# OpenVectorAI/CoFHE

Measured on AMD Instinct MI355X. Metric: ciphertext-ops/sec + HBM GB/s (% roofline), 128x128 matadd, higher is better.
Workload: dtype u32; 1 GPU; ciphertext_matadd 128x128 per GPU (C2), security 128, k 128, |Delta| = 2088 bits, valid ciphertexts of random plaintexts; elements_per_gpu=16384, parallelism=row-shard x1, collective=none

## Files before the change

### __graft_entry__.py

```python
import json
import os
import subprocess
import sys

ROOT = os.path.dirname(os.path.abspath(__file__))
CSRC = os.path.join(ROOT, "cofhe_amd", "csrc")
LIB = os.path.join(ROOT, "cofhe_amd", "libcofhe_hip.so")
HIP_SOURCES = ["cofhe_hip.hip", "abi.hip", "kernels.hpp", "wire.hip", "shard.hip", "wide.hip", "ctx.hpp", "lane.hpp", "mp.hpp", "qf.hpp",
               "form_io.hpp", "layout.hpp", "wide.hpp", "qfw.hpp", "comb.hip", "comb.hpp"]
HIP_OBJECTS = [("part0", "cofhe_hip.hip", ["-DCOFHE_PART=0"]), ("part1", "cofhe_hip.hip", ["-DCOFHE_PART=1"]),
               ("part2", "cofhe_hip.hip", ["-DCOFHE_PART=2"]), ("abi", "abi.hip", []), ("wire", "wire.hip", []), ("shard", "shard.hip", []),
               ("wide", "wide.hip", []), ("comb", "comb.hip", [])]


def _stale(target, deps):
    if not os.path.exists(target):
        return True
    t = os.path.getmtime(target)
    return any(os.path.getmtime(d) > t for d in deps)


def build_library(src_dir, obj_dir, lib, extra_flags=()) -> None:
    hipcc = os.environ.get("HIPCC", "/opt/rocm/bin/hipcc")
    flags = ["--offload-arch=gfx950", "-O2", "-std=c++17", "-fPIC", "-Wno-unused-value"] + list(extra_flags)
    os.makedirs(obj_dir, exist_ok=True)
    jobs = []
    for name, src, extra in HIP_OBJECTS:
        obj = os.path.join(obj_dir, name + ".o")
        jobs.append((obj, subprocess.Popen([hipcc] + flags + extra + ["-c", os.path.join(src_dir, src), "-o", obj], cwd=ROOT)))
    for obj, pr in jobs:
        if pr.wait() != 0:
            raise subprocess.CalledProcessError(pr.returncode, "hipcc -c -> " + obj)
    subprocess.check_call([hipcc, "--offload-arch=gfx950", "-shared", "-fPIC", "-o", lib] + [o for o, _ in jobs] + ["-ldl"], cwd=ROOT)


def build() -> None:
    deps = [os.path.join(CSRC, f) for f in HIP_SOURCES] + [os.path.join(ROOT, "include", "cofhe_hip.h")]
    if _stale(LIB, deps):
        build_library(CSRC, os.path.join(CSRC, "obj"), LIB)
    odir = os.path.join(ROOT, "oracle")
    if _stale(os.path.join(odir, "libcofhe_oracle.so"),
              [os.path.join(odir, "cofhe_oracle.hpp"), os.path.join(odir, "cofhe_oracle_c.cpp")]):
        subprocess.check_call(["make", "-C", odir])
    hdir = os.path.join(ROOT, "cofhe_amd", "host")
    exe = os.path.join(hdir, "local_bench")
    if _stale(exe, [os.path.join(hdir, f) for f in ("local_bench.cpp", "hip_cryptosystem.hpp", "smpc_local.hpp", "tensor.hpp")] + [LIB]):
        subprocess.check_call(["g++", "-std=c++17", "-O2", "-I/opt/conda/include", "-o", exe,
                               os.path.join(hdir, "local_bench.cpp"), "-L" + os.path.join(ROOT, "cofhe_amd"),
                               "-lcofhe_hip", "-l:libgmp.so.10", "-Wl,-rpath,$ORIGIN/.."], cwd=hdir)
    gdir = os.path.join(ROOT, "tests", "gpu_kernels")
    gso = os.path.join(gdir, "liblehmer_gpu.so")
    if _stale(gso, [os.path.join(gdir, "lehmer_gpu.hip"), os.path.join(CSRC, "mp.hpp"), os.path.join(CSRC, "lane.hpp")]):
        subprocess.check_call([os.environ.get("HIPCC", "/opt/rocm/bin/hipcc"), "--offload-arch=gfx950", "-O2", "-std=c++17", "-fPIC", "-shared",
                               "-Wno-unused-value", "-o", gso, os.path.join(gdir, "lehmer_gpu.hip")], cwd=ROOT)
    sys.path.insert(0, ROOT)
    import cofhe_amd
    cofhe_amd.load_library()


def smoke() -> None:
    sys.path.insert(0, ROOT)
    sys.path.insert(0, os.path.join(ROOT, "tests"))
    from cofhe_amd import Engine
    import oracle_lib as O

    def hx(s):
        return -int(s[1:], 16) if s.startswith("-") else int(s, 16)

    g = os.path.join(ROOT, "tests", "golden")
    prm = json.load(open(os.path.join(g, "params_s128_k128.json")))
    vec = json.load(open(os.path.join(g, "vectors_s128_k128.json")))
    d = hx(prm["delta"])
    eng = Engine(d, device=0)
    v = vec["add_valid"]
    t1, t2 = bytes.fromhex(v["ct1"]), bytes.fromhex(v["ct2"])
    out = eng.add_ciphertext_tensors(t1, t2)
    assert out == bytes.fromhex(v["out"]), "HIP add != golden"
    assert out == O.add(d, t1, t2), "HIP add != oracle"
    v = vec["scal_2d"]
    out = eng.scal_ciphertext_tensors(bytes.fromhex(v["s"]), bytes.fromhex(v["cts"]), bytes.fromhex(v["zero"]))
    assert out == bytes.fromhex(v["out"]), "HIP scal matmul != golden"
    print("smoke ok: add_ciphertext_tensors and scal_ciphertext_tensors match golden vectors and oracle")


if __name__ == "__main__":
    build()
    if len(sys.argv) > 1 and sys.argv[1] == "smoke":
        smoke()
```

### cofhe_amd/csrc/mp.hpp

```cpp
#pragma once
#include "lane.hpp"

namespace cofhe {

#if defined(COFHE_HOSTSIM)
struct SimStats { long batches, batch_steps, divsteps, muls, divrems, resolves, bits_gained; };
inline SimStats g_stats;
#define CF_STAT(x) do { if (c.gl == 0) { x; } } while (0)
#else
#define CF_STAT(x) do { } while (0)
#endif

CF_DEV uint32_t opaque(uint32_t v) {
#if defined(COFHE_HOSTSIM)
    asm volatile("" : "+r"(v));
#else
    asm volatile("" : "+v"(v));
#endif
    return v;
}

template <int P>
struct Mp {
    uint32_t v[P][CH];
};

template <int P>
struct SMp {
    Mp<P> m;
    int neg;
};

template <int P>
CF_DEV void mp_zero(Mp<P> &x) {
    CF_UNROLL for (int p = 0; p < P; p++) CF_UNROLL for (int j = 0; j < CH; j++) x.v[p][j] = 0;
}

template <int P>
CF_DEV void mp_set_word(Ctx &c, Mp<P> &x, uint32_t w) {
    mp_zero(x);
    x.v[0][0] = (c.gl == 0) ? w : 0u;
}

template <int Q, int P>
CF_DEV Mp<Q> mp_resize(const Mp<P> &x) {
    Mp<Q> r;
    CF_UNROLL for (int p = 0; p < Q; p++)
        CF_UNROLL for (int j = 0; j < CH; j++) r.v[p][j] = (p < P) ? x.v[p < P ? p : 0][j] : 0u;
    return r;
}

template <int P>
CF_DEV void mp_select(Mp<P> &r, bool take_y, const Mp<P> &x, const Mp<P> &y) {
    CF_UNROLL for (int p = 0; p < P; p++)
        CF_UNROLL for (int j = 0; j < CH; j++) r.v[p][j] = take_y ? y.v[p][j] : x.v[p][j];
}

template <int P>
CF_DEV void mp_swap(Mp<P> &x, Mp<P> &y) {
    CF_UNROLL for (int p = 0; p < P; p++)
        CF_UNROLL for (int j = 0; j < CH; j++) {
            uint32_t t = x.v[p][j];
            x.v[p][j] = y.v[p][j];
            y.v[p][j] = t;
        }
}

template <int P>
CF_DEV bool mp_is_zero(Ctx &c, const Mp<P> &x) {
    uint32_t o = 0;
    CF_UNROLL for (int p = 0; p < P; p++) CF_UNROLL for (int j = 0; j < CH; j++) o |= x.v[p][j];
    return ballot8(c, o != 0) == 0;
}

template <int P>
CF_DEV bool mp_high_planes_zero(Ctx &c, const Mp<P> &x, int from) {
    uint32_t o = 0;
    CF_UNROLL for (int p = 0; p < P; p++)
        CF_UNROLL for (int j = 0; j < CH; j++) o |= (p >= from) ? x.v[p][j] : 0u;
    return ballot8(c, o != 0) == 0;
}

template <int P>
CF_DEV bool mp_is_word(Ctx &c, const Mp<P> &x, uint32_t w) {
    uint32_t o = 0;
    CF_UNROLL for (int p = 0; p < P; p++)
        CF_UNROLL for (int j = 0; j < CH; j++) {
            uint32_t want = (p == 0 && j == 0 && c.gl == 0) ? w : 0u;
            o |= x.v[p][j] ^ want;
        }
    return ballot8(c, o != 0) == 0;
}

template <int P>
CF_DEV int mp_bitlen(Ctx &c, const Mp<P> &x) {
    uint32_t top = x.v[0][0], idx = 0;
    CF_UNROLL for (int p = 0; p < P; p++)
        CF_UNROLL for (int j = 0; j < CH; j++) {
            if (p == 0 && j == 0) continue;
            const uint32_t w = x.v[p][j];
            top = w ? w : top;
            idx = w ? (uint32_t)(p * PLIMBS + j) : idx;
        }
    const uint32_t best = top ? (idx + (uint32_t)c.gl * CH) * 32u + 32u - (uint32_t)clz32(top) : 0u;
    return (int)group_max(c, best);
}

template <int P>
CF_DEV int mp_cmp(Ctx &c, const Mp<P> &x, const Mp<P> &y) {
    uint32_t key = 0;
    CF_UNROLL for (int p = 0; p < P; p++)
        CF_UNROLL for (int j = 0; j < CH; j++) {
            uint32_t a = x.v[p][j], b = y.v[p][j];
            uint32_t k = ((uint32_t)(p * PLIMBS + c.gl * CH + j + 1) << 1) | (a > b ? 1u : 0u);
            key = (a != b) ? k : key;
        }
    uint32_t m = group_max(c, key);
    return m == 0 ? 0 : ((m & 1) ? 1 : -1);
}

template <int P>
CF_DEV uint32_t mp_get_limb(Ctx &c, const Mp<P> &x, int idx) {
    if (idx < 0 || idx >= P * PLIMBS) return 0;
    int p = idx / PLIMBS, w = idx % PLIMBS;
    int lane = w / CH, j = w % CH;
    uint32_t cand = 0;
    CF_UNROLL for (int pp = 0; pp < P; pp++)
        CF_UNROLL for (int jj = 0; jj < CH; jj++) cand = (pp == p && jj == j) ? x.v[pp][jj] : cand;
    return bcast(c, cand, lane);
}

template <int P>
CF_DEV uint64_t mp_bits64(Ctx &c, const Mp<P> &x, int pos) {
    int i0 = pos >> 5, o = pos & 31;
    uint32_t l0 = mp_get_limb(c, x, i0), l1 = mp_get_limb(c, x, i0 + 1), l2 = mp_get_limb(c, x, i0 + 2);
    uint64_t lo = ((uint64_t)l1 << 32) | l0;
    return o ? ((lo >> o) | ((uint64_t)l2 << (64 - o))) : lo;
}
template <int P>
CF_DEV uint32_t mp_bits32(Ctx &c, const Mp<P> &x, int pos) {
    int i0 = pos >> 5, o = pos & 31;
    uint32_t l0 = mp_get_limb(c, x, i0), l1 = mp_get_limb(c, x, i0 + 1);
    return o ? ((l0 >> o) | (l1 << (32 - o))) : l0;
}

template <int P>
CF_DEV uint32_t mp_resolve(Ctx &c, Mp<P> &r, const uint32_t (&hi)[P]) {
    uint32_t plane_word = 0, plane_bit = 0;
    CF_STAT(g_stats.resolves += P);
    CF_UNROLL for (int p = 0; p < P; p++) {
        uint32_t inc = shfl_up1(c, hi[p], plane_word);
        uint64_t t = (uint64_t)r.v[p][0] + inc + ((c.gl == 0) ? plane_bit : 0u);
        r.v[p][0] = (uint32_t)t;
        uint32_t cy = (uint32_t)(t >> 32);
        uint32_t all = r.v[p][0];
        CF_UNROLL for (int j = 1; j < CH; j++) {
            t = (uint64_t)r.v[p][j] + cy;
            r.v[p][j] = (uint32_t)t;
            cy = (uint32_t)(t >> 32);
// ... 60 lines not shown
    uint64_t t[CH];
    CF_UNROLL for (int j = 0; j < CH; j++)
        t[j] = (uint64_t)A * x[j] + (uint64_t)B * (NOTY ? (uint32_t)~y[j] : y[j]);
    uint32_t prev = cin;
#if defined(COFHE_HOSTSIM)
    uint32_t carry = 0;
    CF_UNROLL for (int j = 0; j < CH; j++) {
        const uint64_t s = (uint64_t)(uint32_t)t[j] + prev + carry;
        r[j] = (uint32_t)s;
        carry = (uint32_t)(s >> 32);
        prev = (uint32_t)(t[j] >> 32);
    }
    return prev + carry;
#else
    static_assert(CH == 5, "carry chain written for 5 limbs per lane");
    uint32_t l0 = (uint32_t)t[0], l1 = (uint32_t)t[1], l2 = (uint32_t)t[2], l3 = (uint32_t)t[3], l4 = (uint32_t)t[4];
    const uint32_t h0 = (uint32_t)(t[0] >> 32), h1 = (uint32_t)(t[1] >> 32), h2 = (uint32_t)(t[2] >> 32),
                   h3 = (uint32_t)(t[3] >> 32);
    uint32_t h4 = (uint32_t)(t[4] >> 32);
    asm("v_add_co_u32 %0, vcc, %0, %6\n\t"
        "s_nop 1\n\t"
        "v_addc_co_u32 %1, vcc, %1, %7, vcc\n\t"
        "s_nop 1\n\t"
        "v_addc_co_u32 %2, vcc, %2, %8, vcc\n\t"
        "s_nop 1\n\t"
        "v_addc_co_u32 %3, vcc, %3, %9, vcc\n\t"
        "s_nop 1\n\t"
        "v_addc_co_u32 %4, vcc, %4, %10, vcc\n\t"
        "s_nop 1\n\t"
        "v_addc_co_u32 %5, vcc, 0, %5, vcc"
        : "+v"(l0), "+v"(l1), "+v"(l2), "+v"(l3), "+v"(l4), "+v"(h4)
        : "v"(prev), "v"(h0), "v"(h1), "v"(h2), "v"(h3)
        : "vcc");
    r[0] = l0; r[1] = l1; r[2] = l2; r[3] = l3; r[4] = l4;
    return h4;
#endif
}


template <int P>
CF_DEV uint32_t mp_lincomb_add(Ctx &c, Mp<P> &r, uint32_t A, const Mp<P> &x, uint32_t B, const Mp<P> &y) {
    uint32_t hi[P];
    CF_UNROLL for (int p = 0; p < P; p++) hi[p] = lincomb_plane<false>(r.v[p], A, x.v[p], B, y.v[p], 0u);
    return mp_resolve_sparse(c, r, hi);
}

template <int P>
CF_DEV void mp_lincomb_sub(Ctx &c, Mp<P> &r, uint32_t A, const Mp<P> &x, uint32_t B, const Mp<P> &y) {
    uint32_t hi[P];
    CF_UNROLL for (int p = 0; p < P; p++)
        hi[p] = lincomb_plane<true>(r.v[p], A, x.v[p], B, y.v[p], (p == 0 && c.gl == 0) ? B : 0u);
    (void)mp_resolve(c, r, hi);
}

template <int P>
CF_DEV uint32_t mp_lincomb_sub_carry(Ctx &c, Mp<P> &r, uint32_t A, const Mp<P> &x, uint32_t B, const Mp<P> &y) {
    uint32_t hi[P];
    CF_UNROLL for (int p = 0; p < P; p++)
        hi[p] = lincomb_plane<true>(r.v[p], A, x.v[p], B, y.v[p], (p == 0 && c.gl == 0) ? B : 0u);
    return mp_resolve(c, r, hi);
}

template <int P>
CF_DEV void mp_sub(Ctx &c, Mp<P> &r, const Mp<P> &x, const Mp<P> &y) {
    mp_lincomb_sub(c, r, 1u, x, 1u, y);
}

template <int P>
CF_DEV Mp<P> mp_shl(Ctx &c, const Mp<P> &x, int n) {
    uint32_t *s = c.scratch();
    CF_UNROLL for (int p = 0; p < P; p++)
        CF_UNROLL for (int j = 0; j < CH; j++) s[p * PLIMBS + c.gl * CH + j] = x.v[p][j];
    group_sync(c);
    int w = n >> 5, o = n & 31;
    Mp<P> y;
    CF_UNROLL for (int p = 0; p < P; p++)
        CF_UNROLL for (int j = 0; j < CH; j++) {
            int i = p * PLIMBS + c.gl * CH + j - w;
            uint32_t a = (i >= 0 && i < P * PLIMBS) ? s[i >= 0 && i < P * PLIMBS ? i : 0] : 0u;
            uint32_t b = (i - 1 >= 0 && i - 1 < P * PLIMBS) ? s[i - 1 >= 0 && i - 1 < P * PLIMBS ? i - 1 : 0] : 0u;
            y.v[p][j] = o ? ((a << o) | (b >> (32 - o))) : a;
        }
    group_sync(c);
    return y;
}

template <int P>
CF_DEV Mp<P> mp_shr(Ctx &c, const Mp<P> &x, int n) {
    uint32_t *s = c.scratch();
    CF_UNROLL for (int p = 0; p < P; p++)
        CF_UNROLL for (int j = 0; j < CH; j++) s[p * PLIMBS + c.gl * CH + j] = x.v[p][j];
    group_sync(c);
    int w = n >> 5, o = n & 31;
    Mp<P> y;
    CF_UNROLL for (int p = 0; p < P; p++)
        CF_UNROLL for (int j = 0; j < CH; j++) {
            int i = p * PLIMBS + c.gl * CH + j + w;
            uint32_t a = (i < P * PLIMBS) ? s[i < P * PLIMBS ? i : 0] : 0u;
            uint32_t b = (i + 1 < P * PLIMBS) ? s[i + 1 < P * PLIMBS ? i + 1 : 0] : 0u;
            y.v[p][j] = o ? ((a >> o) | (b << (32 - o))) : a;
        }
    group_sync(c);
    return y;
}

template <int P>
CF_DEV Mp<P> mp_shr_small(Ctx &c, const Mp<P> &x, int n) {
    Mp<P> y;
    uint32_t above = 0;
    const uint32_t ls = (uint32_t)(32 - n) & 31u;
    const uint32_t keep = n ? 0xFFFFFFFFu : 0u;
    CF_UNROLL for (int p = P - 1; p >= 0; p--) {
        uint32_t nxt = shfl_down1(c, x.v[p][0], above);
        CF_UNROLL for (int j = 0; j < CH; j++) {
            uint32_t up = (j + 1 < CH) ? x.v[p][j + 1 < CH ? j + 1 : 0] : nxt;
            y.v[p][j] = (x.v[p][j] >> n) | ((up << ls) & keep);
        }
        above = bcast_first(c, x.v[p][0]);
    }
    return y;
}
template <int P>
CF_DEV Mp<P> mp_shr1(Ctx &c, const Mp<P> &x) { return mp_shr_small(c, x, 1); }

CF_DEV void chunk_mac(uint32_t (&w)[2 * CH + 1], const uint32_t (&x)[CH], const uint32_t (&y)[CH]) {
    CF_UNROLL for (int i = 0; i < CH; i++) {
        uint32_t cy = 0;
        CF_UNROLL for (int j = 0; j < CH; j++) {
            uint64_t m = (uint64_t)x[i] * y[j] + w[i + j] + cy;
            w[i + j] = (uint32_t)m;
            cy = (uint32_t)(m >> 32);
        }
        CF_UNROLL for (int k = i + CH; k < 2 * CH + 1; k++) {
            uint64_t m = (uint64_t)w[k] + cy;
            w[k] = (uint32_t)m;
            cy = (uint32_t)(m >> 32);
        }
    }
}
template <int P, int Q>
CF_DEV Mp<P + Q> mp_mul(Ctx &c, const Mp<P> &x, const Mp<Q> &y) {
    constexpr int R = P + Q;
    CF_STAT(g_stats.muls += P * Q);
    static_assert(R * PLIMBS <= SCRATCH_WORDS && R * G * (CH + 1) <= SCRATCH_WORDS, "scratch too small");
    uint32_t *s = c.scratch();
    CF_UNROLL for (int p = 0; p < P; p++)
        CF_UNROLL for (int j = 0; j < CH; j++) s[p * PLIMBS + c.gl * CH + j] = x.v[p][j];
    CF_UNROLL for (int p = 0; p < Q; p++)
        CF_UNROLL for (int j = 0; j < CH; j++) s[(P + p) * PLIMBS + c.gl * CH + j] = y.v[p][j];
    group_sync(c);
    uint32_t w[R][2 * CH + 1];
    CF_UNROLL for (int p = 0; p < R; p++) CF_UNROLL for (int i = 0; i < 2 * CH + 1; i++) w[p][i] = 0;
    const int ybits = mp_bitlen(c, y);
    CF_UNROLL for (int px = 0; px < P; px++) {
        CF_UNROLL for (int py = 0; py < Q; py++) {
            int ky = (ybits - py * PLIMBS * 32 + CH * 32 - 1) / (CH * 32);
            ky = ky < 0 ? 0 : (ky > G ? G : ky);
            uint32_t cur[2 * CH + 1];
            CF_UNROLL for (int i = 0; i < 2 * CH + 1; i++) cur[i] = w[px + py][i];
            for (int k = 0; k < ky; k++) {
                const bool sw = (k == c.gl + 1);
                CF_UNROLL for (int i = 0; i < 2 * CH + 1; i++) {
                    w[px + py][i] = sw ? cur[i] : w[px + py][i];
                    cur[i] = sw ? w[px + py + 1][i] : cur[i];
                }
                const int lx = (c.gl - k) & (G - 1);
                uint32_t xc[CH], yc[CH];
                CF_UNROLL for (int j = 0; j < CH; j++) {
                    xc[j] = s[(px * G + lx) * CH + j];
                    yc[j] = s[P * PLIMBS + (py * G + k) * CH + j];
                }
                chunk_mac(cur, xc, yc);
            }
            const bool never = (c.gl + 1 >= ky);
            CF_UNROLL for (int i = 0; i < 2 * CH + 1; i++) {
                w[px + py][i] = never ? cur[i] : w[px + py][i];
                w[px + py + 1][i] = never ? w[px + py + 1][i] : cur[i];
            }
        }
    }
    group_sync(c);
    CF_UNROLL for (int p = 0; p < R; p++)
        CF_UNROLL for (int i = 0; i < CH + 1; i++) s[(p * G + c.gl) * (CH + 1) + i] = w[p][CH + i];
    group_sync(c);
    Mp<R> r;
    uint32_t hi[R];
    CF_UNROLL for (int p = 0; p < R; p++) {
        int cc = p * G + c.gl;
        uint32_t cy = 0;
        CF_UNROLL for (int j = 0; j < CH; j++) {
            uint32_t up = (cc >= 1) ? s[(cc >= 1 ? cc - 1 : 0) * (CH + 1) + j] : 0u;
            uint32_t ov = (j == 0 && cc >= 2) ? s[(cc >= 2 ? cc - 2 : 0) * (CH + 1) + CH] : 0u;
            uint64_t t = (uint64_t)w[p][j] + up + ov + cy;
            r.v[p][j] = (uint32_t)t;
            cy = (uint32_t)(t >> 32);
        }
        hi[p] = cy;
    }
    group_sync(c);
    (void)mp_resolve_sparse(c, r, hi);
    return r;
}

CF_DEV uint64_t div64_lower(uint64_t n, uint64_t d) {
    double q = (double)(n & ~0x7FFull) / (double)d;
    uint64_t t = (uint64_t)q;
    return t > 0 ? t - 1 : 0;
}

template <int PN, int PD>
CF_DEV uint32_t mp_quot_digit(Ctx &c, const Mp<PN> &num, int nb, const Mp<PD> &den, int db, int &sh) {
    int npos = nb > 64 ? nb - 64 : 0;
    int dpos = db > 32 ? db - 32 : 0;
    uint64_t nt = mp_bits64(c, num, npos);
    uint64_t dt = (uint64_t)mp_bits32(c, den, dpos) + (dpos > 0 ? 1u : 0u);
    int e = npos - dpos;
    uint64_t t;
    if (CF_UNLIKELY(dt == 0)) {
        CF_STATUS(c, CF_ST_DIV_CAP);
        sh = 0;
        return 1;
    }
    if (dpos == 0 && npos == 0) {
        t = nt / dt;
    } else {
        t = div64_lower(nt, dt);
    }
    if (e < 0) {
        t = (-e >= 64) ? 0 : (t >> (-e));
        e = 0;
    }
    int extra = 33 - __builtin_clzll(t | 1);
    if (extra > 0) {
        t >>= extra;
        e += extra;
    }
    sh = e;
    if (t == 0) {
        sh = 0;
        return 1;
    }
    return (uint32_t)t;
}

template <int PN, int PD>
CF_DEV void mp_divrem_cons(Ctx &c, Mp<PN> &num, const Mp<PD> &den, Mp<PN> &quot) {
    static_assert(PN >= PD, "numerator must be at least as wide as the divisor");
    mp_zero(quot);
    const Mp<PN> dw = mp_resize<PN>(den);
    const int db = mp_bitlen(c, den);
    if (db == 0) {
        CF_STATUS(c, CF_ST_DIV_CAP);
        return;
    }
    for (int guard = 0;; guard++) {
        if (guard > PN * PLIMBS * 32 / 28 + 2) {
            CF_STATUS(c, CF_ST_DIV_CAP);
            break;
        }
        int nb = mp_bitlen(c, num);
        if (nb < db) break;
        if (nb == db && mp_cmp(c, num, dw) < 0) break;
        int sh;
        CF_STAT(g_stats.divsteps++);
        uint32_t qd = mp_quot_digit(c, num, nb, den, db, sh);
        Mp<PN> ds = sh ? mp_shl(c, dw, sh) : dw;
        mp_lincomb_sub(c, num, 1u, num, qd, ds);
        Mp<PN> qa;
        int i0 = sh >> 5, o = sh & 31;
        uint32_t lo = qd << o, hiw = o ? (qd >> (32 - o)) : 0u;
        CF_UNROLL for (int p = 0; p < PN; p++)
            CF_UNROLL for (int j = 0; j < CH; j++) {
                int i = p * PLIMBS + c.gl * CH + j;
                qa.v[p][j] = (i == i0) ? lo : ((i == i0 + 1) ? hiw : 0u);
            }
        (void)mp_add(c, quot, quot, qa);
    }
}

struct WordDiv {
    uint32_t w;
    uint64_t m;
};
CF_DEV uint64_t umulhi64(uint64_t a, uint64_t b) {
#if defined(COFHE_HOSTSIM)
    return (uint64_t)(((unsigned __int128)a * b) >> 64);
#else
    return __umul64hi(a, b);
#endif
}
CF_DEV WordDiv worddiv_make(uint32_t w) {
    WordDiv d;
    d.w = w;
    d.m = ~0ull / w;
    return d;
}
CF_DEV uint64_t worddiv_divmod(const WordDiv &d, uint64_t t, uint32_t &rem) {
    uint64_t q = umulhi64(t, d.m);
    uint64_t r = t - q * d.w;
    while (r >= d.w) {
        r -= d.w;
        q++;
    }
    rem = (uint32_t)r;
    return q;
}
CF_DEV uint32_t worddiv_mulmod(const WordDiv &d, uint32_t a, uint32_t b) {
    uint32_t r;
    (void)worddiv_divmod(d, (uint64_t)a * b, r);
    return r;
}
CF_DEV uint32_t worddiv_addmod(const WordDiv &d, uint32_t a, uint32_t b) {
    uint64_t t = (uint64_t)a + b;
    return (uint32_t)(t >= d.w ? t - d.w : t);
}

template <int P>
CF_DEV uint32_t mp_mod_word(Ctx &c, const Mp<P> &x, const WordDiv &d) {
    uint32_t rem;
    uint32_t two32 = (uint32_t)(0x100000000ull % d.w);
    uint32_t beta = 1;
    CF_UNROLL for (int j = 0; j < CH; j++) beta = worddiv_mulmod(d, beta, two32);
    uint32_t total = 0;
    CF_UNROLL for (int p = P - 1; p >= 0; p--) {
        uint32_t r = 0;
        CF_UNROLL for (int j = CH - 1; j >= 0; j--) {
            (void)worddiv_divmod(d, ((uint64_t)r << 32) | x.v[p][j], rem);
            r = rem;
        }
        uint32_t val = r, wgt = beta;
        CF_UNROLL for (int st = 1; st < G; st <<= 1) {
            uint32_t ov = shfl(c, val, c.gl + st), ow = shfl(c, wgt, c.gl + st);
            bool has = (c.gl + st) < G;
            uint32_t nv = worddiv_addmod(d, worddiv_mulmod(d, ov, wgt), val);
            uint32_t nw = worddiv_mulmod(d, wgt, ow);
            val = has ? nv : val;
            wgt = has ? nw : wgt;
        }
        uint32_t plane_val = bcast_first(c, val), plane_w = bcast_first(c, wgt);
        total = worddiv_addmod(d, worddiv_mulmod(d, total, plane_w), plane_val);
    }
    return total;
}

constexpr uint32_t PRIMORIAL23 = 223092870u;
struct PrimorialWeights { uint32_t w[PLIMBS]; };
constexpr PrimorialWeights primorial_weights() {
    PrimorialWeights t{};
    uint64_t v = 1;
    for (int i = 0; i < PLIMBS; i++) {
        t.w[i] = (uint32_t)v;
        v = (v << 32) % PRIMORIAL23;
    }
    return t;
}
#if defined(COFHE_HOSTSIM)
static constexpr PrimorialWeights PRIMORIAL_W = primorial_weights();
#else
__device__ static constexpr PrimorialWeights PRIMORIAL_W = primorial_weights();
#endif
CF_DEV uint32_t mp_mod_primorial(Ctx &c, const Mp<1> &x) {
    uint64_t acc = 0;
    CF_UNROLL for (int j = 0; j < CH; j++) acc += (uint64_t)x.v[0][j] * PRIMORIAL_W.w[c.gl * CH + j];
    uint32_t v = (uint32_t)(acc % PRIMORIAL23);
    v += shfl_xor1(c, v);
    v += shfl_xor2(c, v);
    v += shfl_mirror(c, v);
    return v % PRIMORIAL23;
}

struct ModW {
    WordDiv dv;
    uint32_t w16[2 * CH];
    uint32_t lanew;
    uint32_t planew;
};
CF_DEV ModW modw_make(Ctx &c, uint32_t W) {
    ModW mw;
    mw.dv = worddiv_make(W);
    uint32_t rem;
    mw.w16[0] = 1u % W;
    CF_UNROLL for (int i = 1; i < 2 * CH; i++) {
        (void)worddiv_divmod(mw.dv, (uint64_t)mw.w16[i - 1] << 16, rem);
        mw.w16[i] = rem;
    }
    (void)worddiv_divmod(mw.dv, (uint64_t)mw.w16[2 * CH - 1] << 16, rem);
    const uint32_t p1 = rem;
    const uint32_t p2 = worddiv_mulmod(mw.dv, p1, p1), p4 = worddiv_mulmod(mw.dv, p2, p2);
    static_assert(G == 8, "lane weights written for 8 lanes per group");
    uint32_t lw = (c.gl & 1) ? p1 : mw.w16[0];
    lw = (c.gl & 2) ? worddiv_mulmod(mw.dv, lw, p2) : lw;
    lw = (c.gl & 4) ? worddiv_mulmod(mw.dv, lw, p4) : lw;
    mw.lanew = lw;
    mw.planew = worddiv_mulmod(mw.dv, p4, p4);
    return mw;
}
template <int P>
CF_DEV uint32_t mp_mod_word_fast(Ctx &c, const Mp<P> &x, const ModW &mw) {
    uint32_t total = 0, rem;
    CF_UNROLL for (int p = P - 1; p >= 0; p--) {
        uint64_t acc = 0;
        CF_UNROLL for (int j = 0; j < CH; j++)
            acc += (uint64_t)(x.v[p][j] & 0xFFFFu) * mw.w16[2 * j] + (uint64_t)(x.v[p][j] >> 16) * mw.w16[2 * j + 1];
        (void)worddiv_divmod(mw.dv, acc, rem);
        uint32_t v = worddiv_mulmod(mw.dv, rem, mw.lanew);
        v = worddiv_addmod(mw.dv, v, shfl_xor1(c, v));
        v = worddiv_addmod(mw.dv, v, shfl_xor2(c, v));
        v = worddiv_addmod(mw.dv, v, shfl_mirror(c, v));
        total = worddiv_addmod(mw.dv, worddiv_mulmod(mw.dv, total, mw.planew), v);
    }
    return total;
}
template <int P>
CF_DEV uint32_t mp_divrem_word(Ctx &c, Mp<P> &num, const WordDiv &d) {
    uint32_t rem;
    uint32_t two32 = (uint32_t)(0x100000000ull % d.w);
    uint32_t beta = 1;
    CF_UNROLL for (int j = 0; j < CH; j++) beta = worddiv_mulmod(d, beta, two32);
    uint32_t above = 0;
    CF_UNROLL for (int p = P - 1; p >= 0; p--) {
        uint32_t r = 0;
        CF_UNROLL for (int j = CH - 1; j >= 0; j--) {
            (void)worddiv_divmod(d, ((uint64_t)r << 32) | num.v[p][j], rem);
            r = rem;
        }
        uint32_t val = r, wgt = beta;
        CF_UNROLL for (int st = 1; st < G; st <<= 1) {
            uint32_t ov = shfl(c, val, c.gl + st), ow = shfl(c, wgt, c.gl + st);
            bool has = (c.gl + st) < G;
            uint32_t nv = worddiv_addmod(d, worddiv_mulmod(d, ov, wgt), val);
            uint32_t nw = worddiv_mulmod(d, wgt, ow);
            val = has ? nv : val;
            wgt = has ? nw : wgt;
        }
        uint32_t hv = shfl_down1(c, val, 0u), hw = shfl_down1(c, wgt, 1u);
        uint32_t h = worddiv_addmod(d, worddiv_mulmod(d, above, hw), hv);
        uint32_t rr = h;
        CF_UNROLL for (int j = CH - 1; j >= 0; j--) {
            uint64_t q = worddiv_divmod(d, ((uint64_t)rr << 32) | num.v[p][j], rem);
            num.v[p][j] = (uint32_t)q;
            rr = rem;
        }
        uint32_t pv = bcast_first(c, val), pw = bcast_first(c, wgt);
        above = worddiv_addmod(d, worddiv_mulmod(d, above, pw), pv);
    }
    return above;
}

template <int PN>
CF_DEV void mp_divrem_norm(Ctx &c, Mp<PN> &num, const Mp<1> &den, int db, Mp<PN> &quot) {
    static_assert(2 * PN * PLIMBS <= SCRATCH_WORDS, "scratch too small");
    mp_zero(quot);
    const int nb = mp_bitlen(c, num);
    if (nb < db) return;
    const int s = PLIMBS * 32 - db;
    const Mp<1> D = s ? mp_shl(c, den, s) : den;
    const uint32_t d39 = bcast_last(c, D.v[0][CH - 1]), d38 = bcast_last(c, D.v[0][CH - 2]);
    const double rd = 1.0 / ((double)d39 * 4294967296.0 + (double)d38);
    uint32_t *sn = c.scratch(), *sq = sn + PN * PLIMBS;
    CF_UNROLL for (int p = 0; p < PN; p++)
        CF_UNROLL for (int j = 0; j < CH; j++) {
            sn[p * PLIMBS + c.gl * CH + j] = num.v[p][j];
            sq[p * PLIMBS + c.gl * CH + j] = 0u;
        }
    group_sync(c);
    const int sw = s >> 5, sb = s & 31;
    auto limb = [&](int k) -> uint32_t {
        const int i = k - sw;
        const uint32_t a = (i >= 0 && i < PN * PLIMBS) ? sn[(i >= 0 && i < PN * PLIMBS) ? i : 0] : 0u;
        const uint32_t b = (i >= 1 && i <= PN * PLIMBS) ? sn[(i >= 1 && i <= PN * PLIMBS) ? i - 1 : 0] : 0u;
        return sb ? ((a << sb) | (b >> (32 - sb))) : a;
    };
    const int K = (nb + s - 1) >> 5;
    Mp<1> S;
    CF_UNROLL for (int j = 0; j < CH; j++) S.v[0][j] = limb(K - (PLIMBS - 1) + c.gl * CH + j);
    uint32_t top = 0;
    for (int k = K - (PLIMBS - 1);; k--) {
        CF_STAT(g_stats.divsteps++);
        const uint32_t l39 = bcast_last(c, S.v[0][CH - 1]), l38 = bcast_last(c, S.v[0][CH - 2]);
        double x = (((double)top * 4294967296.0 + (double)l39) * 4294967296.0 + (double)l38) * rd;
        x += x * 1.7763568394002505e-15;
        uint64_t qd = (uint64_t)x;
        if (qd > 0xFFFFFFFFull) qd = 0xFFFFFFFFull;
        if (CF_LIKELY(qd != 0)) {
            Mp<1> T;
            const uint32_t cw = mp_lincomb_sub_carry(c, T, 1u, S, (uint32_t)qd, D);
            int64_t nt = (int64_t)top + (int64_t)cw - (int64_t)qd;
            S = T;
            for (int fix = 0; CF_UNLIKELY(nt < 0) && fix < 4; fix++) {
                CF_FLAG(8u);
                nt += (int64_t)mp_add(c, S, S, D);
                qd--;
            }
        }
        if (c.gl == 0) sq[k] = (uint32_t)qd;
        if (k == 0) break;
        top = bcast_last(c, S.v[0][CH - 1]);
        const uint32_t up = shfl_up1(c, S.v[0][CH - 1], limb(k - 1));
        CF_UNROLL for (int j = CH - 1; j >= 1; j--) S.v[0][j] = S.v[0][j - 1];
        S.v[0][0] = up;
    }
    group_sync(c);
    CF_UNROLL for (int p = 0; p < PN; p++)
        CF_UNROLL for (int j = 0; j < CH; j++) quot.v[p][j] = sq[p * PLIMBS + c.gl * CH + j];
    group_sync(c);
    const Mp<1> R = s ? mp_shr(c, S, s) : S;
    num = mp_resize<PN>(R);
}

template <int PN, int PD>
CF_DEV void mp_divrem(Ctx &c, Mp<PN> &num, const Mp<PD> &den, Mp<PN> &quot) {
    static_assert(PN >= PD, "numerator must be at least as wide as the divisor");
    CF_STAT(g_stats.divrems++);
    const int db = mp_bitlen(c, den);
    if (CF_UNLIKELY(db == 0)) {
        CF_STATUS(c, CF_ST_DIV_CAP);
        mp_zero(quot);
        return;
    }
    if (db <= 32) {
        WordDiv d = worddiv_make(mp_get_limb(c, den, 0));
        quot = num;
        uint32_t r = mp_divrem_word(c, quot, d);
        mp_set_word(c, num, r);
        return;
    }
    if constexpr (PD == 1) {
        mp_divrem_norm(c, num, den, db, quot);
        return;
    }
    if (db < 64) {
        mp_divrem_cons(c, num, den, quot);
        return;
    }
    mp_zero(quot);
    const int nb = mp_bitlen(c, num);
    if (nb < db) return;
    uint32_t *s = c.scratch();
    CF_UNROLL for (int p = 0; p < PD; p++)
        CF_UNROLL for (int j = 0; j < CH; j++) s[p * PLIMBS + c.gl * CH + j] = den.v[p][j];
    group_sync(c);
    const uint64_t d64 = mp_bits64(c, den, db - 64);
    const double rd = 1.0 / (double)d64;
    for (int jq = (nb - db) / 32; jq >= 0; jq--) {
        CF_STAT(g_stats.divsteps++);
        const int pos = db - 64 + 32 * jq;
        const uint64_t hi64 = mp_bits64(c, num, pos + 32);
        const uint32_t lo32 = mp_bits32(c, num, pos);
        double x = ((double)hi64 * 4294967296.0 + (double)lo32) * rd;
        x += x * 1.7763568394002505e-15;
        uint64_t qd = (uint64_t)x;
        if (qd > 0xFFFFFFFFull) qd = 0xFFFFFFFFull;
        if (qd != 0) {
            Mp<PN> ds;
            CF_UNROLL for (int p = 0; p < PN; p++)
                CF_UNROLL for (int j = 0; j < CH; j++) {
                    int i = p * PLIMBS + c.gl * CH + j - jq;
                    bool ok = i >= 0 && i < PD * PLIMBS;
                    ds.v[p][j] = ok ? s[ok ? i : 0] : 0u;
                }
            mp_lincomb_sub(c, num, 1u, num, (uint32_t)qd, ds);
            for (int fix = 0; fix < 4 && ballot8(c, c.gl == G - 1 && (num.v[PN - 1][CH - 1] >> 31)) != 0; fix++) {
                (void)mp_add(c, num, num, ds);
                qd--;
            }
        }
        CF_UNROLL for (int p = 0; p < PN; p++)
            CF_UNROLL for (int j = 0; j < CH; j++)
                quot.v[p][j] = (p * PLIMBS + c.gl * CH + j == jq) ? (uint32_t)qd : quot.v[p][j];
    }
    group_sync(c);
}

template <int PN, int PQ>
CF_DEV void mp_divexact(Ctx &c, const Mp<PN> &num, const Mp<1> &den, Mp<PQ> &quot, int nq) {
    static_assert((PN + PQ) * PLIMBS <= SCRATCH_WORDS, "scratch too small");
    mp_zero(quot);
    if (nq <= 0) return;
    if (nq > PQ * PLIMBS) nq = PQ * PLIMBS;
    const uint32_t d0raw = bcast_first(c, den.v[0][0]);
    if (CF_UNLIKELY(d0raw == 0)) {
        Mp<PN> rem = num, q;
        mp_divrem(c, rem, den, q);
        quot = mp_resize<PQ>(q);
        return;
    }
    const int tz = __builtin_ctz(d0raw);
    const Mp<1> D = mp_shr_small(c, den, tz);
    const Mp<PN> Nn = mp_shr_small(c, num, tz);
    const uint32_t d0 = d0raw >> tz | (tz ? bcast_first(c, den.v[0][1]) << (32 - tz) : 0u);
    uint32_t dinv = d0;
    CF_UNROLL for (int i = 0; i < 4; i++) dinv *= 2u - d0 * dinv;
    uint32_t *sn = c.scratch(), *sq = sn + PN * PLIMBS;
    CF_UNROLL for (int p = 0; p < PN; p++)
        CF_UNROLL for (int j = 0; j < CH; j++) sn[p * PLIMBS + c.gl * CH + j] = Nn.v[p][j];
    CF_UNROLL for (int p = 0; p < PQ; p++)
        CF_UNROLL for (int j = 0; j < CH; j++) sq[p * PLIMBS + c.gl * CH + j] = 0u;
    group_sync(c);
    Mp<1> S;
    CF_UNROLL for (int j = 0; j < CH; j++) S.v[0][j] = Nn.v[0][j];
    int64_t adj = 0;
    auto high = [&](int k) -> uint32_t { return (PLIMBS + k < PN * PLIMBS) ? sn[(PLIMBS + k < PN * PLIMBS) ? PLIMBS + k : 0] : 0u; };
    const uint64_t d64 = ((uint64_t)bcast_first(c, D.v[0][1]) << 32) | d0;
    uint64_t dinv64 = dinv;
    dinv64 *= 2ull - d64 * dinv64;
    int i = 0;
    for (; i + 1 < nq; i += 2) {
        CF_STAT(g_stats.divsteps += 2);
        const uint64_t s01 = ((uint64_t)bcast_first(c, S.v[0][1]) << 32) | bcast_first(c, S.v[0][0]);
        const uint64_t q = s01 * dinv64;
        const uint32_t q0 = (uint32_t)q, q1 = (uint32_t)(q >> 32);
        uint32_t r1[CH];
        const uint32_t hi1 = lincomb_plane<true>(r1, 1u, S.v[0], q0, D.v[0], c.gl == 0 ? q0 : 0u);
        const int64_t v1 = (int64_t)high(i) + adj + (int64_t)bcast_last(c, hi1) - (int64_t)q0;
        const int64_t adj1 = v1 >> 32;
        const uint32_t inc = shfl_up1(c, hi1, 0u);
        const uint32_t r0 = r1[0] + inc;
        const uint32_t bit = r0 < inc ? 1u : 0u;
        uint32_t s2[CH];
        s2[CH - 1] = shfl_down1(c, r0, (uint32_t)v1);
        CF_UNROLL for (int j = 0; j + 1 < CH; j++) s2[j] = r1[j + 1];
        Mp<1> T;
        uint32_t hi2[1];
        hi2[0] = lincomb_plane<true>(T.v[0], 1u, s2, q1, D.v[0], c.gl == 0 ? q1 : bit);
        const uint32_t cw = mp_resolve(c, T, hi2);
        const int64_t v2 = (int64_t)high(i + 1) + adj1 + (int64_t)cw - (int64_t)q1;
        adj = v2 >> 32;
        const uint32_t up = shfl_down1(c, T.v[0][0], (uint32_t)v2);
        CF_UNROLL for (int j = 0; j + 1 < CH; j++) S.v[0][j] = T.v[0][j + 1];
        S.v[0][CH - 1] = up;
        if (c.gl == 0) {
            sq[i] = q0;
            sq[i + 1] = q1;
        }
    }
    for (; i < nq; i++) {
        CF_STAT(g_stats.divsteps++);
        const uint32_t q = bcast_first(c, S.v[0][0]) * dinv;
        Mp<1> T;
        const uint32_t cw = mp_lincomb_sub_carry(c, T, 1u, S, q, D);
        const int64_t v = (int64_t)high(i) + adj + (int64_t)cw - (int64_t)q;
        adj = v >> 32;
        const uint32_t up = shfl_down1(c, T.v[0][0], (uint32_t)v);
        CF_UNROLL for (int j = 0; j + 1 < CH; j++) S.v[0][j] = T.v[0][j + 1];
        S.v[0][CH - 1] = up;
        if (c.gl == 0) sq[i] = q;
    }
    group_sync(c);
    CF_UNROLL for (int p = 0; p < PQ; p++)
        CF_UNROLL for (int j = 0; j < CH; j++) quot.v[p][j] = sq[p * PLIMBS + c.gl * CH + j];
    group_sync(c);
}

template <int P>
CF_DEV void smp_add(Ctx &c, SMp<P> &r, const SMp<P> &x, const SMp<P> &y) {
    if (x.neg == y.neg) {
        (void)mp_add(c, r.m, x.m, y.m);
        r.neg = x.neg;
    } else {
        int cm = mp_cmp(c, x.m, y.m);
        if (cm >= 0) {
            Mp<P> t;
            mp_sub(c, t, x.m, y.m);
            r.m = t;
            r.neg = cm == 0 ? 0 : x.neg;
        } else {
            Mp<P> t;
            mp_sub(c, t, y.m, x.m);
            r.m = t;
            r.neg = y.neg;
        }
    }
}
template <int P>
CF_DEV void smp_sub(Ctx &c, SMp<P> &r, const SMp<P> &x, const SMp<P> &y) {
    SMp<P> ny = y;
    ny.neg ^= 1;
    smp_add(c, r, x, ny);
}
template <int P, int Q>
CF_DEV SMp<P + Q> smp_mul(Ctx &c, const SMp<P> &x, const SMp<Q> &y) {
    SMp<P + Q> r;
    r.m = mp_mul(c, x.m, y.m);
    r.neg = x.neg ^ y.neg;
    return r;
}

CF_DEV void mp_bits64_pair(Ctx &c, const Mp<1> &x, const Mp<1> &y, int pos, uint64_t &xh, uint64_t &yh) {
    uint32_t *s = c.scratch();
    CF_UNROLL for (int j = 0; j < CH; j++) {
        s[c.gl * CH + j] = x.v[0][j];
        s[PLIMBS + c.gl * CH + j] = y.v[0][j];
    }
    s[2 * PLIMBS + c.gl] = 0u;
    group_sync(c);
    const int i0 = pos >> 5, o = pos & 31;
    const int i1 = i0 + 1 < PLIMBS ? i0 + 1 : 2 * PLIMBS, i2 = i0 + 2 < PLIMBS ? i0 + 2 : 2 * PLIMBS;
    const uint32_t x0 = s[i0], x1 = s[i1 < PLIMBS ? i1 : 2 * PLIMBS], x2 = s[i2 < PLIMBS ? i2 : 2 * PLIMBS];
    const uint32_t y0 = s[PLIMBS + i0], y1 = s[i1 < PLIMBS ? PLIMBS + i1 : 2 * PLIMBS],
                   y2 = s[i2 < PLIMBS ? PLIMBS + i2 : 2 * PLIMBS];
    group_sync(c);
    const uint64_t xl = ((uint64_t)x1 << 32) | x0, yl = ((uint64_t)y1 << 32) | y0;
    xh = o ? ((xl >> o) | ((uint64_t)x2 << (64 - o))) : xl;
    yh = o ? ((yl >> o) | ((uint64_t)y2 << (64 - o))) : yl;
}

template <int P>
struct Euclid {
    Mp<P> x, y, ux, uy;
    int sx, sy;
};

CF_DEV float u64_to_float(uint64_t v) {
    uint32_t hi = (uint32_t)(v >> 32), lo = (uint32_t)v;
#if defined(COFHE_HOSTSIM)
    asm volatile("" : "+r"(hi));
#else
    asm volatile("" : "+v"(hi));
#endif
    return (float)hi * 4294967296.0f + (float)lo;
}
CF_DEV uint32_t f32_to_u32_sat(float x) {
#if defined(COFHE_HOSTSIM)
    if (!(x >= 1.0f)) return 0u;
// ... 388 lines not shown
```

### cofhe_amd/csrc/qf.hpp

```cpp
#pragma once
#include "mp.hpp"

namespace cofhe {

struct QForm {
    Mp<1> a;
    Mp<1> bm;
    int bneg;
    Mp<2> c;
};

template <int P>
CF_DEV void qf_reduce(Ctx &c, Mp<P> &a, SMp<P> &b, Mp<P> &cc) {
    for (int guard = 0;; guard++) {
        if (CF_UNLIKELY(guard > 4 * P * PLIMBS * 32)) {
            CF_STATUS(c, CF_ST_REDUCE_CAP);
            return;
        }
        int cm = mp_cmp(c, b.m, a);
        if (cm > 0 || (cm == 0 && b.neg)) {
            Mp<P> two_a;
            (void)mp_add(c, two_a, a, a);
            if (mp_cmp(c, b.m, two_a) < 0) {
                Mp<P> t;
                mp_sub(c, t, two_a, b.m);
                Mp<P> u;
                (void)mp_add(c, u, cc, a);
                mp_sub(c, cc, u, b.m);
                b.m = t;
                b.neg ^= 1;
            } else {
                int nb = mp_bitlen(c, b.m), db = mp_bitlen(c, two_a), sh;
                uint32_t qd = mp_quot_digit(c, b.m, nb, two_a, db, sh);
                Mp<P> ds = sh ? mp_shl(c, two_a, sh) : two_a;
                Mp<P> nbm;
                mp_lincomb_sub(c, nbm, 1u, b.m, qd, ds);
                Mp<P> half;
                uint32_t top = mp_add(c, half, b.m, nbm);
                half = mp_shr1(c, half);
                if (top) {
                    Mp<P> tb;
                    mp_zero(tb);
                    tb.v[P - 1][CH - 1] = (c.gl == G - 1) ? 0x80000000u : 0u;
                    (void)mp_add(c, half, half, tb);
                }
                Mp<P> hs = sh ? mp_shl(c, half, sh) : half;
                mp_lincomb_sub(c, cc, 1u, cc, qd, hs);
                b.m = nbm;
            }
            continue;
        }
        int ac = mp_cmp(c, a, cc);
        if (ac > 0) {
            mp_swap(a, cc);
            b.neg ^= 1;
            continue;
        }
        if (mp_is_zero(c, b.m)) b.neg = 0;
        if (ac == 0 && b.neg) b.neg = 0;
        return;
    }
}

template <int P>
CF_DEV Mp<1> smod(Ctx &c, const SMp<P> &t, const Mp<1> &v) {
    Mp<P> rem = t.m, q;
    mp_divrem(c, rem, v, q);
    Mp<1> r = mp_resize<1>(rem);
    if (t.neg && !mp_is_zero(c, r)) {
        Mp<1> u;
        mp_sub(c, u, v, r);
        r = u;
    }
    return r;
}

template <int QP, int P>
CF_DEV SMp<QP> sdiv_exact(Ctx &c, const SMp<P> &n, const Mp<1> &v) {
    SMp<QP> r;
    const int nb = mp_bitlen(c, n.m), vb = mp_bitlen(c, v);
    mp_divexact(c, n.m, v, r.m, nb == 0 ? 0 : (nb - vb + 1 + 31) / 32);
    r.neg = n.neg;
    return r;
}

CF_DEV void nucomp_m12(Ctx &c, SMp<1> &M1, SMp<2> &M2, const Mp<1> &R, const SMp<1> &C, const Mp<1> &v1,
                       const Mp<1> &v2, const SMp<1> &m, const SMp<1> &s, const Mp<2> &c2d) {
    SMp<1> Rs{R, 0};
    SMp<1> v2s{v2, 0};
    SMp<2> t1 = smp_mul(c, v2s, Rs);
    SMp<2> t2 = smp_mul(c, m, C);
    SMp<2> n1;
    smp_sub(c, n1, t1, t2);
    M1 = sdiv_exact<1>(c, n1, v1);
    SMp<2> t3 = smp_mul(c, s, Rs);
    SMp<2> c2s{c2d, 0};
    SMp<3> t4w = smp_mul(c, c2s, C);
    SMp<2> t4{mp_resize<2>(t4w.m), t4w.neg};
    SMp<2> n2;
    smp_add(c, n2, t3, t4);
    M2 = sdiv_exact<2>(c, n2, v1);
}

CF_DEV SMp<2> nucomp_dot(Ctx &c, const Mp<1> &R, const SMp<1> &C, const SMp<1> &M1, const SMp<2> &M2) {
    SMp<1> Rs{R, 0};
    SMp<2> p1 = smp_mul(c, Rs, M1);
    SMp<3> p2w = smp_mul(c, C, M2);
    SMp<2> p2{mp_resize<2>(p2w.m), p2w.neg};
    SMp<2> r;
    smp_add(c, r, p1, p2);
    return r;
}

struct QDisc {
    const uint32_t *absdelta;
    int half_dbits;
};

template <int WG>
CF_DEV void qf_euclid(Ctx &c, Euclid<1> &e, int stop_bits) {
#if defined(COFHE_HOSTSIM)
    if (WG != 0 && c.wg) {
        euclid_run_wg(c, e, stop_bits);
        return;
    }
#else
    if (WG != 0) {
        euclid_run_wg(c, e, stop_bits);
        return;
    }
#endif
    euclid_run(c, e, stop_bits);
}

CF_DEV void word_xgcd(uint32_t m, uint32_t a, uint32_t &g, uint32_t &inv) {
    uint32_t r0 = m, r1 = a;
    int64_t t0 = 0, t1 = 1;
    for (int it = 0; it < 64 && r1 != 0; it++) {
        const uint32_t q = r0 / r1, r2 = r0 - q * r1;
        const int64_t t2 = t0 - (int64_t)q * t1;
        r0 = r1; r1 = r2;
        t0 = t1; t1 = t2;
    }
    g = r0;
    inv = (uint32_t)(t0 < 0 ? t0 + (int64_t)m : t0);
}
CF_DEV void word_xgcd16(uint32_t m, uint32_t a, uint32_t &g, uint32_t &inv) {
    uint32_t r0 = m, r1 = a;
    int32_t t0 = 0, t1 = 1;
    for (int it = 0; it < 32 && r1 != 0; it++) {
        uint32_t q = f32_to_u32_sat((float)r0 * fast_rcp((float)r1) * 0.99999905f);
        uint32_t r2 = r0 - q * r1;
        if (r2 >= r1) { r2 -= r1; q++; }
        const int32_t t2 = t0 - (int32_t)q * t1;
        r0 = r1; r1 = r2;
        t0 = t1; t1 = t2;
    }
    g = r0;
    inv = (uint32_t)(t0 < 0 ? t0 + (int32_t)m : t0);
}
CF_DEV_COLD bool qf_word_factor_residue(Ctx &c, Mp<1> &r, Mp<1> &v1, Mp<1> &v2, Mp<2> &c2d, const Mp<1> &d, const SMp<1> &s,
                                        const SMp<1> &m, const SMp<1> &y1) {
    const uint32_t dw = bcast_first(c, d.v[0][0]);
    if (CF_UNLIKELY(mp_bitlen(c, d) > 16)) { CF_FLAG(16u); return false; }
    const WordDiv dv = worddiv_make(dw);
    const ModW mw = modw_make(c, dw * dw);
    uint32_t sd, rem;
    const uint32_t sW = mp_mod_word_fast(c, s.m, mw);
    (void)worddiv_divmod(dv, sW, sd);
    if (sd == 0) {
        Mp<1> q1 = v1, q2 = v2;
        const uint32_t rem1 = mp_divrem_word(c, q1, dv), rem2 = mp_divrem_word(c, q2, dv);
        if (CF_UNLIKELY((rem1 | rem2) != 0)) { CF_FLAG(32u); return false; }
        Mp<2> cd;
        (void)mp_lincomb_add(c, cd, dw, c2d, 0u, c2d);
        Mp<1> rr = r, qq;
        mp_divrem(c, rr, q1, qq);
        r = rr; v1 = q1; v2 = q2; c2d = cd;
        return true;
    }
    uint32_t g = 0, xc = 0;
    word_xgcd16(dw, sd, g, xc);
    const uint32_t r0W = mp_mod_word_fast(c, r, mw), a1W = mp_mod_word_fast(c, v1, mw);
    uint32_t r0rem, a1rem;
    const uint32_t r0q = (uint32_t)worddiv_divmod(dv, r0W, r0rem);
    const uint32_t a1q = (uint32_t)worddiv_divmod(dv, a1W, a1rem);
    uint32_t ga = 0, ainv = 0;
    if (a1q != 0) word_xgcd16(dw, a1q, ga, ainv);
    if (CF_UNLIKELY(!(g == 1 && ga == 1 && r0rem == 0 && a1rem == 0))) {
        CF_FLAG((g != 1 ? 64u : 0u) | (ga != 1 ? 128u : 0u) | ((r0rem | a1rem) != 0 ? 256u : 0u));
        return false;
    }
    (void)worddiv_divmod(mw.dv, (uint64_t)xc * sW, rem);
    const uint32_t y2d = (uint32_t)worddiv_divmod(dv, rem - 1u, rem);
    uint32_t y1d, md, c2w;
    (void)worddiv_divmod(dv, mp_mod_word_fast(c, y1.m, mw), y1d);
    if (y1.neg && y1d) y1d = dw - y1d;
    (void)worddiv_divmod(dv, mp_mod_word_fast(c, m.m, mw), md);
    if (!m.neg && md) md = dw - md;
    (void)worddiv_divmod(dv, mp_mod_word_fast(c, c2d, mw), c2w);
    const uint32_t x2d = s.neg ? dw - xc : xc;
    const uint32_t u = worddiv_mulmod(dv, worddiv_mulmod(dv, y1d, y2d), md);
    const uint32_t v = worddiv_mulmod(dv, x2d, c2w);
    const uint32_t rd = worddiv_addmod(dv, u, v ? dw - v : 0u);
    const uint32_t j = worddiv_mulmod(dv, worddiv_addmod(dv, rd, r0q ? dw - r0q : 0u), ainv);
    Mp<1> T;
    (void)mp_lincomb_add(c, T, 1u, r, j, v1);
    (void)mp_divrem_word(c, T, dv);
    r = T;
    return true;
}
template <int WG = 0, bool WORD_ROUTE = true>
CF_DEV void qf_compose(Ctx &c, QForm &out, const QForm &fa, const QForm &fb, const QDisc &dd) {
    const int half_dbits = dd.half_dbits;
    CF_PHASE(0);
    QForm fbr = fb;
    const bool same = mp_cmp(c, fa.a, fb.a) == 0;
    if (CF_LIKELY(mp_bitlen(c, fb.c) <= PLIMBS * 32 - 110)) {
        const uint32_t M = PRIMORIAL23;
        const uint32_t ra1 = mp_mod_primorial(c, fa.a), ra2 = mp_mod_primorial(c, fb.a);
// ... 310 lines not shown
```

Before: 47.93 million ciphertext-ops/s.

## Use two-limb quotient steps in normalized division and add remainder-only path

Rewrites the normalized long-division loop to produce two 32-bit quotient digits per iteration. Each step estimates the digits from a three-word leading-digit correction and applies both in one fused lincomb pass, so the number of serial division steps and broadcasts roughly halves. Adds an mp_rem path that skips quotient storage and its syncs, used by smod. Also skips multiply passes over zero upper planes of x in mp_mul. The price is more complex estimate and fix-up logic with extra correctness risk.

```diff
diff --git a/__graft_entry__.py b/__graft_entry__.py
--- a/__graft_entry__.py
+++ b/__graft_entry__.py
@@ -49,10 +49,11 @@
                                os.path.join(hdir, "local_bench.cpp"), "-L" + os.path.join(ROOT, "cofhe_amd"),
                                "-lcofhe_hip", "-l:libgmp.so.10", "-Wl,-rpath,$ORIGIN/.."], cwd=hdir)
     gdir = os.path.join(ROOT, "tests", "gpu_kernels")
-    gso = os.path.join(gdir, "liblehmer_gpu.so")
-    if _stale(gso, [os.path.join(gdir, "lehmer_gpu.hip"), os.path.join(CSRC, "mp.hpp"), os.path.join(CSRC, "lane.hpp")]):
-        subprocess.check_call([os.environ.get("HIPCC", "/opt/rocm/bin/hipcc"), "--offload-arch=gfx950", "-O2", "-std=c++17", "-fPIC", "-shared",
-                               "-Wno-unused-value", "-o", gso, os.path.join(gdir, "lehmer_gpu.hip")], cwd=ROOT)
+    for name in ("lehmer_gpu", "divrem_gpu"):
+        gso = os.path.join(gdir, "lib%s.so" % name)
+        if _stale(gso, [os.path.join(gdir, name + ".hip"), os.path.join(CSRC, "mp.hpp"), os.path.join(CSRC, "lane.hpp")]):
+            subprocess.check_call([os.environ.get("HIPCC", "/opt/rocm/bin/hipcc"), "--offload-arch=gfx950", "-O2", "-std=c++17", "-fPIC", "-shared",
+                                   "-Wno-unused-value", "-o", gso, os.path.join(gdir, name + ".hip")], cwd=ROOT)
     sys.path.insert(0, ROOT)
     import cofhe_amd
     cofhe_amd.load_library()
diff --git a/cofhe_amd/csrc/mp.hpp b/cofhe_amd/csrc/mp.hpp
--- a/cofhe_amd/csrc/mp.hpp
+++ b/cofhe_amd/csrc/mp.hpp
@@ -4,7 +4,7 @@
 namespace cofhe {
 
 #if defined(COFHE_HOSTSIM)
-struct SimStats { long batches, batch_steps, divsteps, muls, divrems, resolves, bits_gained; };
+struct SimStats { long batches, batch_steps, divsteps, muls, divrems, resolves, bits_gained, div_lead_fix, div_addback; };
 inline SimStats g_stats;
 #define CF_STAT(x) do { if (c.gl == 0) { x; } } while (0)
 #else
@@ -371,10 +371,13 @@
     uint32_t w[R][2 * CH + 1];
     CF_UNROLL for (int p = 0; p < R; p++) CF_UNROLL for (int i = 0; i < 2 * CH + 1; i++) w[p][i] = 0;
     const int ybits = mp_bitlen(c, y);
+    int xbits = P * PLIMBS * 32;
+    if constexpr (P > 1) xbits = mp_bitlen(c, x);
     CF_UNROLL for (int px = 0; px < P; px++) {
         CF_UNROLL for (int py = 0; py < Q; py++) {
             int ky = (ybits - py * PLIMBS * 32 + CH * 32 - 1) / (CH * 32);
             ky = ky < 0 ? 0 : (ky > G ? G : ky);
+            if (px > 0 && xbits <= px * PLIMBS * 32) ky = 0;
             uint32_t cur[2 * CH + 1];
             CF_UNROLL for (int i = 0; i < 2 * CH + 1; i++) cur[i] = w[px + py][i];
             for (int k = 0; k < ky; k++) {
@@ -666,21 +669,30 @@
     return above;
 }
 
-template <int PN>
-CF_DEV void mp_divrem_norm(Ctx &c, Mp<PN> &num, const Mp<1> &den, int db, Mp<PN> &quot) {
+struct NoQuot {};
+template <typename QT> struct mp_has_quot { static constexpr bool value = true; };
+template <> struct mp_has_quot<NoQuot> { static constexpr bool value = false; };
+
+template <int PN, typename QT>
+CF_DEV void mp_divrem_norm(Ctx &c, Mp<PN> &num, const Mp<1> &den, int db, QT &quot) {
+    constexpr bool QUOT = mp_has_quot<QT>::value;
     static_assert(2 * PN * PLIMBS <= SCRATCH_WORDS, "scratch too small");
-    mp_zero(quot);
+    if constexpr (QUOT) mp_zero(quot);
     const int nb = mp_bitlen(c, num);
     if (nb < db) return;
     const int s = PLIMBS * 32 - db;
     const Mp<1> D = s ? mp_shl(c, den, s) : den;
-    const uint32_t d39 = bcast_last(c, D.v[0][CH - 1]), d38 = bcast_last(c, D.v[0][CH - 2]);
+    uint32_t D1[CH];
+    D1[0] = shfl_up1(c, D.v[0][CH - 1], 0u);
+    CF_UNROLL for (int j = 1; j < CH; j++) D1[j] = D.v[0][j - 1];
+    const uint32_t d39 = bcast_last(c, D.v[0][CH - 1]), d38 = bcast_last(c, D.v[0][CH - 2]), d37 = bcast_last(c, D.v[0][CH - 3]);
+    const uint64_t dlo = ((uint64_t)d38 << 32) | d37;
     const double rd = 1.0 / ((double)d39 * 4294967296.0 + (double)d38);
     uint32_t *sn = c.scratch(), *sq = sn + PN * PLIMBS;
     CF_UNROLL for (int p = 0; p < PN; p++)
         CF_UNROLL for (int j = 0; j < CH; j++) {
             sn[p * PLIMBS + c.gl * CH + j] = num.v[p][j];
-            sq[p * PLIMBS + c.gl * CH + j] = 0u;
+            if constexpr (QUOT) sq[p * PLIMBS + c.gl * CH + j] = 0u;
         }
     group_sync(c);
     const int sw = s >> 5, sb = s & 31;
@@ -691,37 +703,63 @@
         return sb ? ((a << sb) | (b >> (32 - sb))) : a;
     };
     const int K = (nb + s - 1) >> 5;
+    const int k0 = (K - (PLIMBS - 1)) | 1;
     Mp<1> S;
-    CF_UNROLL for (int j = 0; j < CH; j++) S.v[0][j] = limb(K - (PLIMBS - 1) + c.gl * CH + j);
-    uint32_t top = 0;
-    for (int k = K - (PLIMBS - 1);; k--) {
-        CF_STAT(g_stats.divsteps++);
-        const uint32_t l39 = bcast_last(c, S.v[0][CH - 1]), l38 = bcast_last(c, S.v[0][CH - 2]);
-        double x = (((double)top * 4294967296.0 + (double)l39) * 4294967296.0 + (double)l38) * rd;
+    CF_UNROLL for (int j = 0; j < CH; j++) S.v[0][j] = limb(k0 + 1 + c.gl * CH + j);
+    for (int k = k0; k >= 1; k -= 2) {
+        CF_STAT(g_stats.divsteps += 2);
+        const uint32_t v41 = bcast_last(c, S.v[0][CH - 1]), v40 = bcast_last(c, S.v[0][CH - 2]),
+                       v39 = bcast_last(c, S.v[0][CH - 3]), v38 = bcast_last(c, S.v[0][CH - 4]);
+        double x = (((double)v41 * 4294967296.0 + (double)v40) * 4294967296.0 + (double)v39) * rd;
         x += x * 1.7763568394002505e-15;
-        uint64_t qd = (uint64_t)x;
-        if (qd > 0xFFFFFFFFull) qd = 0xFFFFFFFFull;
-        if (CF_LIKELY(qd != 0)) {
-            Mp<1> T;
-            const uint32_t cw = mp_lincomb_sub_carry(c, T, 1u, S, (uint32_t)qd, D);
-            int64_t nt = (int64_t)top + (int64_t)cw - (int64_t)qd;
-            S = T;
+        uint64_t qe = (uint64_t)x;
+        uint32_t q1 = qe > 0xFFFFFFFFull ? 0xFFFFFFFFu : (uint32_t)qe;
+        const uint64_t p0 = (uint64_t)q1 * d37, p1 = (uint64_t)q1 * d38, p2 = (uint64_t)q1 * d39;
+        const uint64_t ml = p0 + (p1 << 32), mh = p2 + (p1 >> 32) + (ml < p0 ? 1u : 0u);
+        const uint64_t vl = ((uint64_t)v39 << 32) | v38, vh = ((uint64_t)v41 << 32) | v40;
+        uint64_t wlo = vl - ml, whi = vh - mh - (vl < ml ? 1u : 0u);
+        if (CF_UNLIKELY((int64_t)whi < 0)) {
+            CF_FLAG(512u);
+            CF_STAT(g_stats.div_lead_fix++);
+            q1--;
+            wlo += dlo;
+            whi += (uint64_t)d39 + (wlo < dlo ? 1u : 0u);
+        }
+        x = (((double)(uint32_t)whi * 4294967296.0 + (double)(uint32_t)(wlo >> 32)) * 4294967296.0 + (double)(uint32_t)wlo) * rd;
+        x += x * 1.7763568394002505e-15;
+        qe = (uint64_t)x;
+        const uint32_t q0 = (qe > 0xFFFFFFFFull || (whi >> 32) != 0) ? 0xFFFFFFFFu : (uint32_t)qe;
+        uint64_t q = ((uint64_t)q1 << 32) | q0;
+        Mp<1> X;
+        X.v[0][0] = shfl_up1(c, S.v[0][CH - 2], limb(k - 1));
+        X.v[0][1] = shfl_up1(c, S.v[0][CH - 1], limb(k));
+        CF_UNROLL for (int j = 2; j < CH; j++) X.v[0][j] = S.v[0][j - 2];
+        if (CF_LIKELY(q != 0)) {
+            uint32_t r1[CH], hi[1];
+            const uint32_t hi1 = lincomb_plane<true>(r1, 1u, X.v[0], q1, D1, c.gl == 0 ? q1 : 0u);
+            hi[0] = lincomb_plane<true>(X.v[0], 1u, r1, q0, D.v[0], shfl_up1(c, hi1, q0));
+            const uint64_t cw = (uint64_t)mp_resolve(c, X, hi) + bcast_last(c, hi1);
+            int64_t nt = (int64_t)(cw + vh - (uint64_t)q1 - (uint64_t)q0 - (uint64_t)q1 * d39);
             for (int fix = 0; CF_UNLIKELY(nt < 0) && fix < 4; fix++) {
                 CF_FLAG(8u);
-                nt += (int64_t)mp_add(c, S, S, D);
-                qd--;
+                CF_STAT(g_stats.div_addback++);
+                nt += (int64_t)mp_add(c, X, X, D);
+                q--;
             }
         }
-        if (c.gl == 0) sq[k] = (uint32_t)qd;
-        if (k == 0) break;
-        top = bcast_last(c, S.v[0][CH - 1]);
-        const uint32_t up = shfl_up1(c, S.v[0][CH - 1], limb(k - 1));
-        CF_UNROLL for (int j = CH - 1; j >= 1; j--) S.v[0][j] = S.v[0][j - 1];
-        S.v[0][0] = up;
-    }
-    group_sync(c);
-    CF_UNROLL for (int p = 0; p < PN; p++)
-        CF_UNROLL for (int j = 0; j < CH; j++) quot.v[p][j] = sq[p * PLIMBS + c.gl * CH + j];
+        S = X;
+        if constexpr (QUOT) {
+            if (c.gl == 0) {
+                sq[k] = (uint32_t)(q >> 32);
+                sq[k - 1] = (uint32_t)q;
+            }
+        }
+    }
+    if constexpr (QUOT) {
+        group_sync(c);
+        CF_UNROLL for (int p = 0; p < PN; p++)
+            CF_UNROLL for (int j = 0; j < CH; j++) quot.v[p][j] = sq[p * PLIMBS + c.gl * CH + j];
+    }
     group_sync(c);
     const Mp<1> R = s ? mp_shr(c, S, s) : S;
     num = mp_resize<PN>(R);
@@ -789,6 +827,23 @@
                 quot.v[p][j] = (p * PLIMBS + c.gl * CH + j == jq) ? (uint32_t)qd : quot.v[p][j];
     }
     group_sync(c);
+}
+
+template <int PN>
+CF_DEV void mp_rem(Ctx &c, Mp<PN> &num, const Mp<1> &den) {
+    CF_STAT(g_stats.divrems++);
+    const int db = mp_bitlen(c, den);
+    if (CF_UNLIKELY(db == 0)) {
+        CF_STATUS(c, CF_ST_DIV_CAP);
+        return;
+    }
+    if (db <= 32) {
+        const WordDiv d = worddiv_make(mp_get_limb(c, den, 0));
+        mp_set_word(c, num, mp_mod_word(c, num, d));
+        return;
+    }
+    NoQuot nq;
+    mp_divrem_norm(c, num, den, db, nq);
 }
 
 template <int PN, int PQ>
diff --git a/cofhe_amd/csrc/qf.hpp b/cofhe_amd/csrc/qf.hpp
--- a/cofhe_amd/csrc/qf.hpp
+++ b/cofhe_amd/csrc/qf.hpp
@@ -64,8 +64,8 @@
 
 template <int P>
 CF_DEV Mp<1> smod(Ctx &c, const SMp<P> &t, const Mp<1> &v) {
-    Mp<P> rem = t.m, q;
-    mp_divrem(c, rem, v, q);
+    Mp<P> rem = t.m;
+    mp_rem(c, rem, v);
     Mp<1> r = mp_resize<1>(rem);
     if (t.neg && !mp_is_zero(c, r)) {
         Mp<1> u;
```

Measured after the change: 48.28 million ciphertext-ops/s (median of 6 runs). About the same (+0.7%).
